# alexkroman/tiny-audio

Measured on AMD Instinct MI355X. Metric: training audio-sec/sec on 10s@16kHz clips, higher is better.
Workload: dtype bf16

## Files before the change

### include/ta355.h

```cpp
#ifndef TA355_H
#define TA355_H

#ifdef __cplusplus
extern "C" {
#endif

#ifndef __HIP_PLATFORM_AMD__
typedef struct ihipStream_t* hipStream_t;
#endif

#define TA_OK 0
#define TA_ERR_ARG 1
#define TA_ERR_LAUNCH 2

int ta_version(void);



long ta_logmel_scratch_floats(int B, int Ls, int n_mels);
int ta_logmel_mel_ranges(const float* melfb, int n_mels, int* mel_ranges, hipStream_t st);
int ta_logmel_f32(const float* wav, const long* lens, int B, int Ls, const float* dft, const float* window,
                  const float* melfb, int n_mels, float* feats, int* mask, float* scratch, const int* mel_ranges, hipStream_t st);

typedef struct {
// ... 199 lines not shown
int ta_lm_forward_loss_ex(const ta_lm_weights* w, const long* ids, const int* src_row, const float* audio,
                          const int* kmask, const int* pos, int B, int L, const int* label_rows,
                          const long* label_targets, int n_label_rows, float loss_scale, float* loss,
                          float* nll_rows, void* logits_out, void* tape, void* ws, long ws_bytes,
                          const ta_lora_dropout* drop, hipStream_t st);
int ta_lm_backward_ex(const ta_lm_weights* w, const int* src_row, const int* kmask, const int* pos, int B, int L,
                      const int* label_rows, int n_label_rows, float* d_audio, long n_audio_rows, float* d_embeds,
                      const ta_lm_lora_grads* lora_grads, const ta_lm_wgrads* wgrads, const long* ids, const void* tape, void* ws,
                      long ws_bytes, const ta_lora_dropout* drop, hipStream_t st);
int ta_lora_dropout_keep(const ta_lora_dropout* drop, int layer, int linear, int M, int in, unsigned char* out, hipStream_t st);


int ta_attention_enc_fwd(const void* qkv, void* out, int B, int heads, int S, hipStream_t st);

int ta_gemm_bf16_nt(const void* A, const void* W, void* C, int M, int N, int K, long lda, int a_rpb, long a_bs,
                    long ldc, int c_rpb, long c_bs, long c_off, const float* bias, const float* residual, int act,
                    int out_bf16, int splits, float* splitk_ws, hipStream_t st);
int ta_gemm_bf16_nt_ex(const void* A, const void* W, void* C, int M, int N, int K, long lda, int a_rpb, long a_bs,
                       long ldc, int c_rpb, long c_bs, long c_off, const float* bias, const float* residual, int act,
                       int out_bf16, int splits, float* splitk_ws, const int* a_idx, const int* seg,
                       const int* krange, hipStream_t st);
typedef struct {
  const void* a2; const void* w2; int k2; long lda2;
  const void* residual_bf16;
  const float* rope_tab; int rope_rows;
  int w_blocked;
  int rope_cols;
} ta_gemm_opts;
int ta_gemm_bf16_nt_opt(const void* A, const void* W, void* C, int M, int N, int K, long lda, int a_rpb, long a_bs,
                        long ldc, int c_rpb, long c_bs, long c_off, const float* bias, const float* residual, int act,
                        int out_bf16, int splits, float* splitk_ws, const int* a_idx, const int* seg,
                        const int* krange, const ta_gemm_opts* opts, hipStream_t st);
long ta_gemm_splitk_ws_bytes(int M, int N, int splits);
int ta_gemm_bf16_nt_grouped(const void* A, const void* W, void* C, int M, int N, int K, const float* bias, int act, int out_bf16,
                            const int* a_idx, const int* seg, const int* krange, int n_groups, long w_stride, long c_stride,
                            hipStream_t st);
long ta_gemm_bf16_tn_ws_bytes(int M, int Ny, int Nx);
int ta_gemm_bf16_tn(const void* Y, const void* X, float* out, int M, int Ny, int Nx, int accumulate, void* ws, long ws_bytes,
                    hipStream_t st);
int ta_profile_gemm(int enable);
int ta_profile_gemm_collect(double* total_ms, double* total_flops, long* launches);
long ta_profile_gemm_log(long* out, long max_rows);
int ta_gemm_reload_knobs(void);

int ta_layernorm_f32(const float* x, const float* w, const float* b, void* y_bf16, float* y_f32,
                     const float* rowscale, int M, int H, float eps, hipStream_t st);
int ta_layernorm_bf16(const void* x_bf16, const float* w, const float* b, void* y_bf16, float* y_f32, const float* rowscale,
                      int M, int H, float eps, hipStream_t st);
int ta_rmsnorm_fwd(const float* x, const float* w, void* y_bf16, float* y_f32, float* rstd, int M, int H,
                   float eps, int act_gelu, hipStream_t st);
int ta_rmsnorm_bwd(const float* dy, const float* x, const float* rstd, const float* w, const float* dres,
                   float* dx_f32, void* dx_bf16, float* dw_accum, int M, int H, int act_gelu, hipStream_t st);
int ta_rmsnorm_fwd_bf16(const void* x_bf16, const float* w, void* y_bf16, float* y_f32, float* rstd, int M, int H, float eps,
                        hipStream_t st);
int ta_rmsnorm_bwd_bf16(const void* dy, int dy_is_bf16, const void* x_bf16, const float* rstd, const float* w,
                        const float* dres, float* dx_f32, void* dx_bf16, int M, int H, hipStream_t st);
int ta_rmsnorm_bwd_bf16s(const void* dy, int dy_is_bf16, const void* x_bf16, const float* rstd, const float* w,
                         const void* dres_bf16, float* dx_f32, void* dx_bf16, int M, int H, hipStream_t st);
int ta_rmsnorm_bwd_dyb(const void* dy_bf16, const float* x, const float* rstd, const float* w, const float* dres, float* dx_f32,
                       void* dx_bf16, int M, int H, hipStream_t st);

int ta_rmsnorm_dw(const void* dy, int dy_is_bf16, const void* x, int x_is_bf16, const float* rstd, float* dw_accum, int M,
                  int H, hipStream_t st);

int ta_attention_fwd(const void* Q, const void* K, const void* VT, void* O, float* LSE, const int* kmask, int B,
                     int Hq, int Hkv, int L, int Lp, int head_dim, int causal, float scale, hipStream_t st);
// ... 66 lines not shown
```

### tiny_audio_amd/csrc/api.hip

```cpp
#include <cstdlib>
#include "common.h"
#include "internal.h"
#include "../../include/ta355.h"

extern "C" int ta_version(void) { return 4; }

#include <algorithm>
#include "host_util.h"


namespace {
struct EncDesc {
  int H, F, L, nh, NM, max_pos, k1;
  float eps;
  const void *conv1_w, *conv2_w;
  const float *conv1_b, *conv2_b, *norm_w, *norm_b;
  const float *rope_cos, *rope_sin, *rope_il, *pos_emb;
  const ta_enc_layer* layers;
  int res_f32;
  bool whisper;
};
EncDesc enc_desc(const ta_encoder_weights* w) {
  return EncDesc{w->hidden, w->ffn, w->n_layers, w->heads, w->n_mels, w->max_pos, 3 * w->n_mels, w->ln_eps, w->conv1_w, w->conv2_w,
                 w->conv1_b, w->conv2_b, w->norm_w, w->norm_b, w->rope_cos, w->rope_sin, w->rope_il, nullptr, w->layers, w->res_f32, false};
// ... 101 lines not shown
                                          void* out_bf16, float* out_f32, void* ws, long ws_bytes, hipStream_t st) {
  return enc_forward(enc_desc(w), feats, B, T, frame_keep, out_bf16, out_f32, ws, ws_bytes, st);
}

namespace {
struct MlpTape { float *h1, *r1, *h2, *r2; bf16_t* a1; size_t bytes; };
MlpTape mlp_tape(const ta_mlp_weights* w, int B, int S, void* base) {
  const int N = (S - w->k) / w->k + 1;
  const long Mp = (long)B * N;
  Carver c(base);
  MlpTape t;
  t.h1 = c.take<float>((size_t)Mp * w->hidden);
  t.r1 = c.take<float>((size_t)Mp);
  t.a1 = c.take<bf16_t>((size_t)Mp * w->hidden);
  t.h2 = c.take<float>((size_t)Mp * w->llm_dim);
  t.r2 = c.take<float>((size_t)Mp);
  t.bytes = c.total();
  return t;
}
struct MlpBwdWs { float *dh2, *da1, *skws, *dgws; bf16_t *dh2b, *dh2T, *a1T, *dh1b, *dh1T, *xsT; size_t bytes; };
MlpBwdWs mlp_bwd_ws(const ta_mlp_weights* w, int B, int S, void* base) {
  const int N = (S - w->k) / w->k + 1, Hd = w->hidden, D = w->llm_dim, In = w->k * w->enc_dim;
  const long Mp = (long)B * N; const int Kp = pad64((int)Mp);
  Carver c(base);
  MlpBwdWs s;
  s.dh2 = c.take<float>((size_t)Mp * D);
  s.dh2b = c.take<bf16_t>((size_t)Mp * D);
  s.dh2T = c.take<bf16_t>((size_t)D * Kp);
  s.a1T = c.take<bf16_t>((size_t)Hd * Kp);
  s.da1 = c.take<float>((size_t)Mp * Hd);
  s.dh1b = c.take<bf16_t>((size_t)Mp * Hd);
  s.dh1T = c.take<bf16_t>((size_t)Hd * Kp);
  s.xsT = c.take<bf16_t>((size_t)In * Kp);
  const int s1 = pick_splits(Hd, In, Kp), s2 = pick_splits(D, Hd, Kp);
  const size_t sk1 = (size_t)ta_gemm_splitk_ws_bytes(Hd, In, s1), sk2 = (size_t)ta_gemm_splitk_ws_bytes(D, Hd, s2);
  s.skws = c.take<float>((sk1 > sk2 ? sk1 : sk2) / 4 + 4);
  s.dgws = c.take<float>((size_t)ta_i_rmsnorm_bwd_ws_floats((int)Mp, Hd > D ? Hd : D));
  s.bytes = c.total();
  return s;
}
}

extern "C" long ta_mlp_tape_bytes(const ta_mlp_weights* w, int B, int S) { return (long)mlp_tape(w, B, S, nullptr).bytes; }
extern "C" long ta_mlp_bwd_workspace_bytes(const ta_mlp_weights* w, int B, int S) {
  return (long)mlp_bwd_ws(w, B, S, nullptr).bytes;
}

extern "C" int ta_mlp_projector_forward(const ta_mlp_weights* w, const void* x, int B, int S, float* y, void* tape,
                                        hipStream_t st) {
  const int k = w->k, E = w->enc_dim, Hd = w->hidden, D = w->llm_dim, In = k * E;
  const int N = (S - k) / k + 1;
  if (B <= 0 || N <= 0) return TA_OK;
  if (In % 64 || Hd % 64 || D % 4 || Hd % 4) return TA_ERR_ARG;
  const int Mp = B * N;
  MlpTape t = mlp_tape(w, B, S, tape);
  RC(ta_gemm_bf16_nt(x, w->w1, t.h1, Mp, Hd, In, In, N, (long)S * E, Hd, 0, 0, 0, nullptr, nullptr, 0, 0, 1, nullptr, st));
  RC(ta_rmsnorm_fwd(t.h1, w->g1, t.a1, nullptr, t.r1, Mp, Hd, w->eps, 1, st));
  RC(gemm(t.a1, w->w2, t.h2, Mp, D, Hd, nullptr, nullptr, 0, 0, st));
  RC(ta_rmsnorm_fwd(t.h2, w->g2, nullptr, y, t.r2, Mp, D, w->eps, 0, st));
  return TA_OK;
}

extern "C" int ta_mlp_projector_backward(const ta_mlp_weights* w, const void* x, int B, int S, const float* dy,
                                         const void* tape, float* dW1, float* dg1, float* dW2, float* dg2, void* ws,
                                         long ws_bytes, hipStream_t st) {
  const int k = w->k, E = w->enc_dim, Hd = w->hidden, D = w->llm_dim, In = k * E;
  const int N = (S - k) / k + 1;
// ... 65 lines not shown
    p.r_post = c.take<float>((size_t)d.M);
    p.gu = c.take<bf16_t>((size_t)d.M * 2 * d.F);
    if (w->lora_rank > 0 || w->train_base) {
      p.xn_s = c.take<bf16_t>((size_t)d.M * d.D); p.xn2_s = c.take<bf16_t>((size_t)d.M * d.D);
      p.act_s = c.take<bf16_t>((size_t)d.M * d.F);
    }
    if (w->lora_rank > 0) {
      p.xa_qkv = c.take<bf16_t>((size_t)d.M * 64); p.xa_o = c.take<bf16_t>((size_t)d.M * 64);
      p.xa_gu = c.take<bf16_t>((size_t)d.M * 64); p.xa_d = c.take<bf16_t>((size_t)d.M * 64);
      auto img = [&](LoraImg& g, int in, int N) {
        g.a = c.take<bf16_t>((size_t)64 * in); g.at = c.take<bf16_t>((size_t)64 * in);
        g.b = c.take<bf16_t>((size_t)64 * N); g.bt = c.take<bf16_t>((size_t)64 * N);
      };
      img(p.i_qkv, d.D, d.NQKV); img(p.i_o, d.nq * d.hd, d.D); img(p.i_gu, d.D, 2 * d.F); img(p.i_d, d.F, d.D);
    }
  }
  t.x_final = c.take<float>((size_t)d.M * d.D);
  t.r_f = c.take<float>((size_t)d.M);
  t.hn = c.take<bf16_t>((size_t)d.M * d.D);
  t.dlogits = c.take<bf16_t>((size_t)(n_lab > 0 ? n_lab : 1) * w->vocab_pad);
  t.bytes = c.total();
  return t;
}
struct LmWs {
  bf16_t *xn, *act, *hl, *dxb, *dact, *dgu, *dao, *dot, *dq, *dk, *dv, *dqkv, *dyB;
  float* lora_part;
  long lp_layer, lp_off[8], lp_size[8]; int lp_chunks[8];
  float *logits, *dhl, *dhn, *dxa, *dxb32, *dxn, *delta, *skws;
  bf16_t *tA, *tB;
  float* wsk;
  size_t bytes;
};
inline int wgrad_splits(int n_out, int k_in, int kp) { return pick_splits(n_out, k_in, kp); }
LmWs lm_ws(const ta_lm_weights* w, int B, int L, int n_lab, void* base) {
  const LmDims d = lm_dims(w, B, L);
  const int nl = n_lab > 0 ? n_lab : 1;
  Carver c(base);
  LmWs s;
  s.xn = c.take<bf16_t>((size_t)d.M * d.D);
  s.act = c.take<bf16_t>((size_t)d.M * d.F);
  s.hl = c.take<bf16_t>((size_t)nl * d.D);
  s.logits = c.take<float>((size_t)nl * w->vocab_pad);
  s.dhl = c.take<float>((size_t)nl * d.D);
  s.dhn = c.take<float>((size_t)d.M * d.D);
  s.dxa = c.take<float>((size_t)d.M * d.D);
  s.dxb32 = c.take<float>((size_t)d.M * d.D);
  s.dxn = c.take<float>((size_t)d.M * d.D);
  s.dxb = c.take<bf16_t>((size_t)d.M * d.D);
  s.dact = c.take<bf16_t>((size_t)d.M * d.F);
  s.dgu = c.take<bf16_t>((size_t)d.M * 2 * d.F);
  s.dao = c.take<bf16_t>((size_t)d.M * d.nq * d.hd);
  s.dot = nullptr;
  s.delta = c.take<float>((size_t)B * d.nq * L);
  s.dq = c.take<bf16_t>((size_t)d.M * d.nq * d.hd);
  s.dk = c.take<bf16_t>((size_t)d.M * d.nkv * d.hd);
  s.dv = c.take<bf16_t>((size_t)d.M * d.nkv * d.hd);
  s.dqkv = c.take<bf16_t>((size_t)d.M * d.NQKV);
  s.dyB = c.take<bf16_t>((size_t)d.M * 64);
  s.lora_part = nullptr; s.lp_layer = 0;
  if (w->lora_rank > 0) {
    const int r = w->lora_rank, bq = d.nq * d.hd;
    const int members[4] = {3, 1, 2, 1}, Ng[4] = {d.NQKV, d.D, 2 * d.F, d.D}, ing[4] = {d.D, bq, d.D, d.F};
    long off = 0;
    for (int g = 0; g < 4; ++g) {
      const int chunks = ta_cdiv((int)d.M, ta_i_lora_tn2_rows((int)d.M, Ng[g], ing[g]));
      s.lp_size[2 * g] = (long)members[g] * r * ing[g]; s.lp_size[2 * g + 1] = (long)Ng[g] * r;
      for (int h = 0; h < 2; ++h) { s.lp_chunks[2 * g + h] = chunks; s.lp_off[2 * g + h] = off; off += s.lp_size[2 * g + h] * chunks; }
    }
    s.lp_layer = off;
    s.lora_part = c.take<float>((size_t)off * w->n_layers);
  }
  const int sp = pick_splits(nl, d.D, w->vocab_pad);
  s.skws = c.take<float>((size_t)ta_gemm_splitk_ws_bytes(nl, d.D, sp) / 4 + 4);
  s.tA = s.tB = nullptr; s.wsk = nullptr;
  if (w->train_base) {
    const int Kp = pad64((int)d.M), Kl = pad64(nl), bq = d.nq * d.hd;
    const size_t a_rows = (size_t)std::max(std::max(2 * d.F, d.NQKV), d.D), b_rows = (size_t)std::max(std::max(d.F, bq), d.D);
    s.tA = c.take<bf16_t>(std::max(a_rows * Kp, (size_t)w->vocab_pad * Kl));
    s.tB = c.take<bf16_t>(std::max(b_rows * Kp, (size_t)d.D * Kl));
    const int shp[4][2] = {{d.NQKV, d.D}, {d.D, bq}, {2 * d.F, d.D}, {d.D, d.F}};
    size_t mx = 0;
    for (auto& q : shp) {
      mx = std::max(mx, (size_t)ta_gemm_splitk_ws_bytes(q[0], q[1], wgrad_splits(q[0], q[1], Kp)));
      mx = std::max(mx, (size_t)ta_gemm_bf16_tn_ws_bytes((int)d.M, q[0], q[1]));
    }
    s.wsk = c.take<float>(mx / 4 + 4);
  }
  s.bytes = c.total();
  return s;
}
}

extern "C" long ta_lm_tape_bytes(const ta_lm_weights* w, int B, int L, int n_label_rows) {
  LmLayerTape store[MAX_LM_LAYERS];
  if (w->n_layers > MAX_LM_LAYERS) return -1;
  return (long)lm_tape(w, B, L, n_label_rows, nullptr, store).bytes;
}
extern "C" long ta_lm_workspace_bytes(const ta_lm_weights* w, int B, int L, int n_label_rows) {
  return (long)lm_ws(w, B, L, n_label_rows, nullptr).bytes;
}

static int lm_layers_forward(const ta_lm_weights* w, const LmDims& d, int B, int L, const int* kmask, const int* pos,
                             LmLayerTape* store, bool alias, float* x_final, LmWs& s, const ta_i_lora_layer_imgs* ext,
                             bf16_t* kcache, bf16_t* vcache, int Lmax, hipStream_t st, const LoraDropDev* drop = nullptr) {
  const int M = (int)d.M;
  const float scale = 1.0f / sqrtf((float)d.hd);
  const bool lora = w->lora_rank > 0;
  const int r = w->lora_rank;
  if (lora && (r < 1 || 3 * r > 64)) return TA_ERR_ARG;
  const int lgm = lora ? (w->lora_groups ? w->lora_groups : 15) : 0;
  ta_gemm_opts kx = opts_none();
  auto lora_fwd = [&](const bf16_t* x, int in, const LoraImg& g, bf16_t* xa, int members, int lj0) -> int {
    if (drop) RC(ta_i_lora_skinny_nt_drop(x, in, g.a, xa, M, LoraDrop{*drop, (unsigned)lj0, r, members}, st));
    else RC(ta_i_lora_skinny_nt(x, in, g.a, xa, M, members * r, st));
    kx = opts_kext(xa, g.b);
    return TA_OK;
// ... 371 lines not shown
```

### tiny_audio_amd/csrc/gemm.hip

```cpp
#include "gemm_common.h"

template <int ACT, bool OUT_BF16, bool HAS_RES, int BMT = 128, bool KEXT = false>
__global__ __launch_bounds__(256, 2) void gemm_nt_kernel(GemmArgs p) {
  constexpr int MI = BMT / 32, WR = BMT / 2;
  __shared__ __attribute__((aligned(16))) char smem[4 * TILE_BYTES];
  const int tid = threadIdx.x, lane = tid & 63, wave = tid >> 6;
  const int wm = wave >> 1, wn = wave & 1;
  const int g = lane >> 4, l15 = lane & 15;

  const int nwg = gridDim.x;
  int bid = blockIdx.x;
  {
    const int q = nwg >> 3, r = nwg & 7, xcd = bid & 7, within = bid >> 3;
    bid = (xcd < r ? xcd * (q + 1) : r * (q + 1) + (xcd - r) * q) + within;
  }
  const int tiles = p.tiles_m * p.tiles_n;
  const int z = bid / tiles;
  int t = bid - z * tiles;
  const int GROUP_M = p.group_m > 0 ? p.group_m : 8;
  const int width = GROUP_M * p.tiles_n;
  const int group = t / width;
  const int first_m = group * GROUP_M;
  const int gsize = min(p.tiles_m - first_m, GROUP_M);
  int pm = first_m + (t % width) % gsize;
// ... 316 lines not shown
    for (int i = 0; i < NB; ++i) glds16_s(wb, w_off[i], base + A_BYTES + i * 8192);
    a_base += a_step; w_base += w_step;
  };
  auto first_dma = [&](const TileCtx& c, int st) {
    const int te = fresh_tid(), lr = te >> 3, clog = (te & 7) ^ ((lr >> 1) & 7);
    if (a_blk) {
#pragma unroll
      for (int i = 0; i < NA; ++i) a_off[i] = (unsigned)((((long)(i * nkt) << 12) + (lr << 6) + clog * 8) * 2);
      a_base = (const char*)(p.A + ((((long)((c.rbase + c.m0) >> 6)) * nkt + c.kb) << 12));
    } else if (p.a_plain) {
#pragma unroll
      for (int i = 0; i < NA; ++i)
        a_off[i] = (unsigned)(((long)(min(c.m0 + i * 64 + lr, c.Mact - 1) - c.m0) * p.lda + clog * 8) * 2);
      a_base = (const char*)(p.A + (long)(c.rbase + c.m0) * p.lda) + (long)c.kb * (BK * 2);
    } else {
#pragma unroll
      for (int i = 0; i < NA; ++i) {
        const int gm = c.rbase + min(c.m0 + i * 64 + lr, c.Mact - 1);
        a_off[i] = (unsigned)(((long)(gm / p.a_rpb) * p.a_bs + (long)(gm % p.a_rpb) * p.lda + clog * 8) * 2);
      }
      a_base = (const char*)p.A + (long)c.kb * (BK * 2);
    }
#pragma unroll
    for (int i = 0; i < NB; ++i) {
      const int gn = min(c.n0 + i * 64 + lr, p.N - 1);
      w_off[i] = p.w_blocked ? (unsigned)(((((long)((gn >> 6) - (c.n0 >> 6)) * nkt) << 12) + ((gn & 63) << 6) + clog * 8) * 2)
                             : (unsigned)(((long)(gn - c.n0) * p.K + clog * 8) * 2);
    }
    w_base = (const char*)c.Wp + (p.w_blocked ? (((long)(c.n0 >> 6) * nkt) << 13) + (long)c.kb * 8192 : ((long)c.n0 * p.K + (long)c.kb * BK) * 2);
    if (c.kb < c.ke) dma_tile(lds_w + st * STAGE);
  };
  constexpr bool GELU = ACT == 1;
  constexpr bool ROPE = ACT == 2;
  auto dma_epi = [&](const TileCtx& c, unsigned base) {
    const int te = fresh_tid();
    if (c.biasp && te < BN2 / 4) {
      const int n = c.n0 + te * 4;
      glds16_s(uniform_ptr((const char*)c.biasp), (unsigned)((n < p.N ? n : p.N - 4) * 4), base + EPI_LDS_BIAS);
    }
    if (GELU && !p.gelu_erf) {
      static_assert(GELU_LUT_N * 8 == 512 * 16, "one 16-B piece per thread");
      glds16_s(uniform_ptr((const char*)kGeluLut), (unsigned)(te * 16), base + EPI_LDS_TAB);
    }
    if (ROPE) {
      const char* rb = uniform_ptr((const char*)p.rope_tab);
#pragma unroll
      for (int i = 0; i < BM2 * 128 / 8192; ++i) {
        const int q = i * 512 + te, r = q >> 3, cch = q & 7;
        const int m = c.rbase + min(c.m0 + r, c.Mact - 1);
        glds16_s(rb, (unsigned)(((m % p.rope_rows) * 32 + ((cch ^ (r & 7)) << 2)) * 4), base + EPI_LDS_TAB + i * 8192);
      }
    }
  };

  const bool res_init = residual_is_start<ACT, OUT_BF16, HAS_RES>(p);
  int h = blockIdx.x;
  TileCtx cur = tile_ctx<BM2, BN2>(p, h, total);
  while (!cur.ok) {
    h += gridDim.x;
    if (h >= total) return;
    cur = tile_ctx<BM2, BN2>(p, h, total);
  }
  int ph = 0;
  first_dma(cur, ph);

  for (;;) {
    f32x4 acc[MI][NT];
    if (res_init) {
      const int te = fresh_tid();
      residual_start<MI, NT>(acc, p, cur.m0 + (te >> 8) * (BM2 / 2) + (te & 15), cur.Mact, cur.rbase, cur.n0 + ((te >> 6) & 3) * (BN2 / 4), (te >> 4) & 3);
    } else {
      zero_acc<MI, NT>(acc);
    }

    asm volatile("s_waitcnt vmcnt(0)" ::: "memory");
    __syncthreads();
    int hn = h + gridDim.x;
    TileCtx nx; nx.ok = 0;
    while (hn < total) {
      nx = tile_ctx<BM2, BN2>(p, hn, total);
      if (nx.ok) break;
      hn += gridDim.x;
    }
    if (lag) __builtin_amdgcn_s_barrier();
    for (int kt = cur.kb; kt < cur.ke; ++kt) {
      const int cs = ((kt - cur.kb) & 1) ^ ph;
      const bool more = kt + 1 < cur.ke;
      const char* S = smem + cs * STAGE;
      const unsigned nxt = lds_w + (cs ^ 1) * STAGE;
      bf16x8 af[MI], bfr[NT];
#pragma unroll
      for (int kk = 0; kk < 2; ++kk) {
        const int ko = kk ? koff1 : koff0;
#pragma unroll
        for (int j = 0; j < NT; ++j) bfr[j] = *(const bf16x8*)(S + b_rd + j * 2048 + ko);
#pragma unroll
        for (int i = 0; i < MI; ++i) af[i] = *(const bf16x8*)(S + a_rd + i * 2048 + ko);
        if (kk == 0) {
          if (more) {
            dma_tile(nxt);
          } else {
            dma_epi(cur, nxt);
          }
// ... 14 lines not shown
        __builtin_amdgcn_sched_barrier(0);
        __builtin_amdgcn_s_barrier();
        __builtin_amdgcn_sched_barrier(0);
      }
    }
    if (!lag) __builtin_amdgcn_s_barrier();

    const int nK = cur.ke - cur.kb;
    const int last = __builtin_amdgcn_readfirstlane(nK > 0 ? (((nK - 1) & 1) ^ ph) : ph);
    const char* els = smem + (last ^ 1) * STAGE;
    if (nK <= 0) {
      dma_epi(cur, lds_w + (last ^ 1) * STAGE);
      asm volatile("s_waitcnt vmcnt(0)" ::: "memory");
      __syncthreads();
    }
    if (nx.ok) first_dma(nx, last);
    const float2* lut = (GELU && !p.gelu_erf) ? (const float2*)(els + EPI_LDS_TAB) : nullptr;

    const int te = fresh_tid();
    const int e_l15 = te & 15, e_g = (te >> 4) & 3, e_wn = (te >> 6) & 3, e_wm = te >> 8;
    char* Cb = (char*)p.C;
    if (p.splits > 1) Cb += (long)cur.z * p.slab_stride * 4;
    const bool wide = epilogue_wide_ok(p);
    const int erow0 = e_wm * (BM2 / 2) + e_l15;
    const bool full = OUT_BF16 && wide && p.c_plain && (!HAS_RES || res_init) && cur.m0 + BM2 <= cur.Mact && cur.n0 + BN2 <= p.N;
    if constexpr (OUT_BF16) {
      if (full) epilogue_tile_full<MI, NT, ACT, true>(acc, p, Cb, cur.m0 + erow0, cur.rbase, cur.n0 + e_wn * (BN2 / 4), e_g, cur.biasp, lut, els, cur.n0, erow0);
    }
    if (full) { }
    else if (res_init)
      epilogue_tile<MI, NT, ACT, OUT_BF16, false, 0, true>(acc, p, Cb, cur.m0 + erow0, cur.Mact, cur.rbase, cur.n0 + e_wn * (BN2 / 4), e_g,
                                                           wide, cur.biasp, lut, els, cur.n0, erow0);
    else
      epilogue_tile<MI, NT, ACT, OUT_BF16, HAS_RES, ((BM2 == 192 || (HAS_RES && !OUT_BF16 && ACT == 0)) ? 1 : 0), true>(acc, p, Cb, cur.m0 + erow0, cur.Mact, cur.rbase,
                                                                                cur.n0 + e_wn * (BN2 / 4), e_g, wide, cur.biasp, lut, els, cur.n0, erow0);
    if (!nx.ok) return;
    cur = nx; h = hn; ph = last;
  }
}



__global__ void splitk_reduce_kernel(const float* __restrict__ slabs, int splits, long slab_stride, const float* add,
                                     float* out, bf16_t* __restrict__ out_bf, long n4) {
  for (long i = (long)blockIdx.x * blockDim.x + threadIdx.x; i < n4; i += (long)gridDim.x * blockDim.x) {
    float4 s = add ? ((const float4*)add)[i] : make_float4(0.f, 0.f, 0.f, 0.f);
    for (int z = 0; z < splits; ++z) {
      const float4 v = ((const float4*)(slabs + (long)z * slab_stride))[i];
      s.x += v.x; s.y += v.y; s.z += v.z; s.w += v.w;
    }
    if (out) ((float4*)out)[i] = s;
    if (out_bf) {
      uint2 o; o.x = pack2bf(s.x, s.y); o.y = pack2bf(s.z, s.w);
      ((uint2*)out_bf)[i] = o;
    }
  }
}

template <int N> __device__ __forceinline__ void wait_vm_lgkm0_n() { asm volatile("s_waitcnt vmcnt(%0) lgkmcnt(0)" ::"n"(N) : "memory"); }
template <int ACT, bool OUT_BF16, bool HAS_RES, bool KEXT = false>
__global__ __launch_bounds__(256) void gemm_nt_kernel_v5(GemmArgs p) {
  constexpr int BM5 = 192, BN5 = 128, NS = 3;
  constexpr int A_BYTES = BM5 * 128, SLOT = (BM5 + BN5) * 128;
  __shared__ __attribute__((aligned(16))) char smem[NS * SLOT];
  const int tid = threadIdx.x, lane = tid & 63, wave = tid >> 6;
  const int wm = wave >> 1, wn = wave & 1;
  const int g = lane >> 4, l15 = lane & 15;
// ... 129 lines not shown
      }
      __builtin_amdgcn_s_setprio(0);
      if (FIRST) advance(); else rslot = nslot;
    };
    for (int kt = 0; kt < nt; ++kt) {
      step(std::true_type{}, af0, bf0, af1, bf1);
      step(std::false_type{}, af1, bf1, af0, bf0);
    }
    asm volatile("s_waitcnt vmcnt(0)" ::: "memory");
  }

  char* Cb = (char*)p.C;
  if (p.splits > 1) Cb += (long)z * p.slab_stride * 4;
  const bool wide = epilogue_wide_ok(p);
  const float2* lut = stage_gelu_lut<ACT, 256>(smem, p, tid, true);
  if (res_init) epilogue_tile<6, 4, ACT, OUT_BF16, false>(acc, p, Cb, m0 + wm * 96 + l15, Mact, rbase, n0 + wn * 64, g, wide, biasp, lut);
  else epilogue_tile<6, 4, ACT, OUT_BF16, HAS_RES, ((HAS_RES && !OUT_BF16) ? 3 : 2)>(acc, p, Cb, m0 + wm * 96 + l15, Mact, rbase, n0 + wn * 64, g, wide, biasp, lut);
}

#include <vector>
namespace {
struct ProfRec { hipEvent_t a, b; double flops; };
bool g_prof_on = false;
std::vector<ProfRec> g_prof;
#define TA_GEMM_LOG_FIELDS 24
bool g_log_on = false;
std::vector<long> g_log;
}

#include <cstdlib>
struct GemmKnobs {
  int variant;
  int gelu_erf;
  void load() {
    auto i = [](const char* n, int d) { const char* v = getenv(n); return (v && *v) ? atoi(v) : d; };
    variant = i("TA355_GEMM_VARIANT", -1);
    gelu_erf = i("TA355_GELU_LUT", 1) == 0;
  }
};
static GemmKnobs& knobs() {
  static GemmKnobs k = [] { GemmKnobs x; x.load(); return x; }();
  return k;
}
void ta_i_reload_decode_knobs();
extern "C" int ta_gemm_reload_knobs(void) { knobs().load(); ta_i_reload_decode_knobs(); return TA_OK; }

static int pick_variant(int M, int N, int K, int splits) {
  const int forced = knobs().variant;
  if (forced >= 0 && forced <= 12 && !(forced >= 6 && forced <= 9) && forced != 11) return forced;
  const double rate[6] = {1.0, TA355_RATE_256x256, TA355_RATE_256x128, TA355_RATE_256x256_PP, TA355_RATE_256x320_PP, TA355_RATE_96x128};
  const int bm[6] = {128, 256, 256, 256, 256, 96}, bn[6] = {128, 256, 128, 256, 320, 128}, slots[6] = {512, 256, 256, 256, 256, 512};
  int best = 0; double best_t = 1e300;
  for (int v = 0; v < 6; ++v) {
    const long tiles = (long)ta_cdiv(M, bm[v]) * ta_cdiv(N, bn[v]) * splits;
    const double rounds = (double)((tiles + slots[v] - 1) / slots[v]);
    const double t = rounds * (double)bm[v] * bn[v] / rate[v] * ((v == 0 || v == 5) ? 2.0 : 1.0);
    if (t < best_t) { best_t = t; best = v; }
  }
  {
    const long tiles = (long)ta_cdiv(M, 192) * ta_cdiv(N, 128) * splits;
    const double t = (double)((tiles + 255) / 256) * 192.0 * 128.0 / TA355_RATE_192x128;
    if (TA355_RATE_192x128 > 0.0 && K / splits >= 2048 && t < best_t) { best_t = t; best = 10; }
  }
  {
    const long tiles = (long)ta_cdiv(M, 192) * ta_cdiv(N, 256) * splits;
    const double t = (double)((tiles + 255) / 256) * 192.0 * 256.0 / TA355_RATE_192x256_PP;
    if (TA355_RATE_192x256_PP > 0.0 && K / splits >= 128 && t < best_t) { best_t = t; best = 12; }
  }
  return best;
}

template <int ACT, bool OUT_BF16, bool HAS_RES, bool KEXT>
static void launch_variant(int variant, bool persist, int grid, int pgrid, const GemmArgs& a, hipStream_t st) {
  if (variant == 0) TA_LAUNCH((gemm_nt_kernel<ACT, OUT_BF16, HAS_RES, 128, KEXT>), dim3(grid), dim3(256), 0, st, a);
  else if (variant == 5) TA_LAUNCH((gemm_nt_kernel<ACT, OUT_BF16, HAS_RES, 96, KEXT>), dim3(grid), dim3(256), 0, st, a);
  else if (variant == 1) TA_LAUNCH((gemm_nt_kernel_v2<256, ACT, OUT_BF16, HAS_RES, false, KEXT>), dim3(grid), dim3(512), 0, st, a);
  else if (variant == 12) TA_LAUNCH((gemm_nt_kernel_v4<256, ACT, OUT_BF16, HAS_RES, 192>), dim3(pgrid), dim3(512), 0, st, a);
  else if (variant == 3 && persist) TA_LAUNCH((gemm_nt_kernel_v4<256, ACT, OUT_BF16, HAS_RES>), dim3(pgrid), dim3(512), 0, st, a);
  else if (variant == 4 && persist) TA_LAUNCH((gemm_nt_kernel_v4<320, ACT, OUT_BF16, HAS_RES>), dim3(pgrid), dim3(512), 0, st, a);
  else if (variant == 3) TA_LAUNCH((gemm_nt_kernel_v2<256, ACT, OUT_BF16, HAS_RES, true, KEXT>), dim3(grid), dim3(512), 0, st, a);
  else if (variant == 4) TA_LAUNCH((gemm_nt_kernel_v2<320, ACT, OUT_BF16, HAS_RES, true, KEXT>), dim3(grid), dim3(512), 0, st, a);
  else if (variant == 10) TA_LAUNCH((gemm_nt_kernel_v5<ACT, OUT_BF16, HAS_RES, KEXT>), dim3(grid), dim3(256), 0, st, a);
  else TA_LAUNCH((gemm_nt_kernel_v2<128, ACT, OUT_BF16, HAS_RES, false, KEXT>), dim3(grid), dim3(512), 0, st, a);
}

template <int ACT, bool OUT_BF16, bool HAS_RES>
static int launch_gemm(GemmArgs a, hipStream_t st) {
  if (a.A2 && ACT != 0) return TA_ERR_ARG;
  int variant = pick_variant(a.M, a.N, a.K, a.splits);
  const bool a_far = !a.a_plain && ((long)(a.M / a.a_rpb + 1) * a.a_bs + a.lda * a.a_rpb) * 2 >= (1L << 32);
  if (variant == 10 && (a.w_blocked || a.a_idx || a_far)) variant = 5;
  if (variant == 12 && (a.a_idx || a_far || a.A2)) variant = 3;
  const int bm = variant == 0 ? 128 : (variant == 5 ? 96 : ((variant == 10 || variant == 12) ? 192 : 256));
  const int bn = variant == 4 ? 320 : ((variant == 1 || variant == 3 || variant == 12) ? 256 : 128);
  a.tiles_m = ta_cdiv(a.M, bm) + ((a.grp_n > 0 && a.seg) ? a.grp_n : 0); a.tiles_n = ta_cdiv(a.N, bn);
  const int grid = a.tiles_m * a.tiles_n * a.splits;
  a.group_m = (variant != 0 && a.tiles_m <= 8) ? a.tiles_m : 0;
  a.wide = (((long)a.N | a.ldc | a.c_off | a.c_bs) & 7) == 0;
  a.gelu_erf = knobs().gelu_erf;
  const bool persist = (variant == 3 || variant == 4) && !a.a_idx && !a.A2 && !a_far;
  static const int ncu = [] { int dev = 0, n = 0; (void)hipGetDevice(&dev); (void)hipDeviceGetAttribute(&n, hipDeviceAttributeMultiprocessorCount, dev); return n > 0 ? n : 256; }();
  const int pgrid = grid < ncu ? grid : ncu;
  ProfRec r;
  if (g_prof_on) {
    if (hipEventCreate(&r.a) != hipSuccess || hipEventCreate(&r.b) != hipSuccess) return TA_ERR_LAUNCH;
    r.flops = 2.0 * (double)a.M * (double)a.N * (double)a.K;
    (void)hipEventRecord(r.a, st);
  }
  if constexpr (ACT == 0) {
    if (a.A2) launch_variant<ACT, OUT_BF16, HAS_RES, true>(variant, persist, grid, pgrid, a, st);
  }
  if (!a.A2) launch_variant<ACT, OUT_BF16, HAS_RES, false>(variant, persist, grid, pgrid, a, st);
  if (g_prof_on) { (void)hipEventRecord(r.b, st); g_prof.push_back(r); }
  if (g_log_on) {
    const long flags = (a.a_idx ? 1 : 0) | (a.seg ? 2 : 0) | (a.krange ? 4 : 0) | (a.A2 ? 8 : 0) | (a.w_blocked ? 16 : 0) | (a.grp_n > 0 ? 32 : 0) |
                       (a.a_plain ? 256 : 0) | (a.c_plain ? 512 : 0);
    const long rec[TA_GEMM_LOG_FIELDS] = {a.M, a.N, a.K, a.lda, a.a_rpb, a.a_bs, a.ldc, a.c_rpb, a.c_bs, a.c_off, ACT, OUT_BF16 ? 1 : 0,
                                          HAS_RES ? 1 : 0, a.res_bf16, a.bias ? 1 : 0, a.splits, a.rope_cols, a.rope_rows, flags, a.K2, variant,
                                          a.grp_n, 0, persist ? 1 : 0};
    g_log.insert(g_log.end(), rec, rec + TA_GEMM_LOG_FIELDS);
  }
  TA_CHECK_LAUNCH();
  return TA_OK;
}

extern "C" int ta_profile_gemm(int enable) {
  g_prof_on = enable == 1;
// ... 143 lines not shown
```

### tiny_audio_amd/csrc/gemm_common.h

```cpp
#pragma once
#include "common.h"
#include "../../include/ta355.h"
#include <type_traits>

struct GemmArgs {
  const bf16_t* A;
  const bf16_t* W;
  void* C;
  const float* bias;
  const float* res;
  int M, N, K;
  long lda; int a_rpb; long a_bs;
  long ldc; int c_rpb; long c_bs; long c_off;
  int tiles_m, tiles_n, splits;
  long slab_stride;
  const int* a_idx;
  const int* seg;
  const int* krange;
  const bf16_t* A2; const bf16_t* W2; int K2; long lda2;
  int res_bf16;
  const float* rope_tab; int rope_rows; int rope_cols;
  int group_m;
  int wide;
  int w_blocked;
  int a_plain, c_plain;
  int gelu_erf;
  int a_blocked;
  int grp_n; long grp_w_stride;
};

#define BM 128
#define BN 128
#define BK 64
#ifndef TA355_RATE_256x256
#define TA355_RATE_256x256 0.9
#define TA355_RATE_256x128 0.5
#define TA355_RATE_256x256_PP 1.40
#define TA355_RATE_96x128 0.93
#define TA355_RATE_192x128 1.1
#define TA355_RATE_192x256_PP 1.15
#define TA355_RATE_256x320_PP 1.42
#endif
#define TILE_BYTES (BM * BK * 2)
#include "gelu_lut.h"

__device__ __forceinline__ void glds16_s(const char* base, unsigned off, unsigned lds) {
  asm volatile("s_mov_b32 m0, %0\n\ts_nop 0\n\tglobal_load_lds_dwordx4 %1, %2" ::"s"(lds), "v"(off), "s"(base) : "memory");
}
__device__ __forceinline__ const char* uniform_ptr(const char* q) {
  const unsigned long v = (unsigned long)q;
  const unsigned lo = __builtin_amdgcn_readfirstlane((unsigned)v), hi = __builtin_amdgcn_readfirstlane((unsigned)(v >> 32));
  return (const char*)(((unsigned long)hi << 32) | lo);
}
__device__ __forceinline__ void glds16(const void* g, void* l) {
  __builtin_amdgcn_global_load_lds((const __attribute__((address_space(1))) void*)g,
                                   (__attribute__((address_space(3))) void*)l, 16, 0, 0);
}

__device__ __forceinline__ float gelu_lut(float x, const float2* lut) {
  float t = fmaf(x, GELU_LUT_SCALE, GELU_LUT_BIAS);
  t = __builtin_amdgcn_fmed3f(t, 0.f, (float)(GELU_LUT_N - 1));
  const float2 e = lut[(int)t];
  return fmaf(e.x, x, e.y);
}
#define EPI_LDS_BIAS 0
#define EPI_LDS_TAB 2048
__device__ __forceinline__ int opaque_sgpr(int v) { asm volatile("" : "+s"(v)); return v; }
template <int NT> struct EpiPre { uint2 r[NT]; };
template <int NT, int ACT, bool OUT_BF16, bool HAS_RES, bool ELS = false>
__device__ __forceinline__ void epilogue_strip(const f32x4* acc, const GemmArgs& p, char* Cb, long roff, int nb, int g, bool wide,
                                               int m, const float* bias, const float2* lut = nullptr, const EpiPre<NT>* pre = nullptr,
                                               bool pre_r = false, const char* els = nullptr, int ecol0 = 0, int erow = 0,
                                               uint2* oret = nullptr, const float4* pref = nullptr) {
  static_assert(ACT >= 0 && ACT <= 2, "epilogue form");
  constexpr int BASE = ACT;
// ... 65 lines not shown
  }
}
template <int MI, int NT, int ACT, bool ELS>
__device__ __forceinline__ void epilogue_tile_full(const f32x4 (*acc)[NT], const GemmArgs& p, char* Cb, int ml0, int rbase, int nb, int g,
                                                   const float* bias, const float2* lut, const char* els, int ecol0, int erow0) {
  static_assert(NT >= 4, "two column pairs per strip");
  const int l15 = ml0 & 15;
  const long own0 = p.c_off + (long)(rbase + ml0) * p.ldc;
  const long step = 16L * p.ldc;
  const int colx = nb + (l15 >> 3) * 32 + 16 * (g & 1) + 8 * (g >> 1);
  char* px = Cb + (p.c_off + (long)(rbase + ml0 - (l15 & 8)) * p.ldc + colx) * 2;
  char* py = px + 16L * p.ldc;
#pragma unroll
  for (int i = 0; i < MI; ++i) {
    uint2 o[NT];
    epilogue_strip<NT, ACT, true, false, ELS>(acc[i], p, Cb, own0 + i * step, nb, g, true, rbase + ml0 + i * 16, bias, lut, nullptr, false, els,
                                              ecol0, erow0 + i * 16, o);
    uint32_t q[2][4];
#pragma unroll
    for (int pp = 0; pp < 2; ++pp) {
      const auto a = __builtin_amdgcn_permlane16_swap(o[2 * pp].x, o[2 * pp + 1].x, false, false);
      const auto b = __builtin_amdgcn_permlane16_swap(o[2 * pp].y, o[2 * pp + 1].y, false, false);
      q[pp][0] = a[0]; q[pp][1] = b[0]; q[pp][2] = a[1]; q[pp][3] = b[1];
    }
    uint32_t x[4], y[4];
#pragma unroll
    for (int d = 0; d < 4; ++d) {
      x[d] = __builtin_amdgcn_update_dpp(q[0][d], q[1][d], 0x128, 0xf, 0xc, false);
      y[d] = __builtin_amdgcn_update_dpp(q[1][d], q[0][d], 0x128, 0xf, 0x3, false);
    }
    *(uint4*)(px + i * step * 2) = make_uint4(x[0], x[1], x[2], x[3]);
    *(uint4*)(py + i * step * 2) = make_uint4(y[0], y[1], y[2], y[3]);
#pragma unroll
    for (int j = 4; j < NT; ++j) *(uint2*)(Cb + (own0 + i * step + nb + j * 16 + g * 4) * 2) = o[j];
  }
}
template <int MI, int NT, int ACT, bool OUT_BF16, bool HAS_RES, int AHEAD = 0, bool ELS = false, int PIN = 0>
__device__ __forceinline__ void epilogue_tile(const f32x4 (*acc)[NT], const GemmArgs& p, char* Cb, int ml0, int Mact, int rbase, int nb,
                                              int g, bool wide, const float* bias, const float2* lut, const char* els = nullptr,
                                              int ecol0 = 0, int erow0 = 0) {
  const int c_rpb_o = opaque_sgpr(p.c_rpb);
  auto row_off = [&](int m) -> long {
    return p.c_off + (p.c_plain ? (long)m * p.ldc : (long)(m / c_rpb_o) * p.c_bs + (long)(m % c_rpb_o) * p.ldc);
  };
  int ncl[NT];
#pragma unroll
  for (int j = 0; j < NT; ++j) {
    const int n = nb + j * 16 + g * 4;
    ncl[j] = n < p.N ? n : p.N - 4;
  }
  const bool pre_r = AHEAD > 0 && HAS_RES && p.res_bf16;
  auto fetch = [&](int i, uint2* dst) {
    int ml = ml0 + i * 16; if (ml >= Mact) ml = Mact - 1;
    const long ro = row_off(rbase + ml);
#pragma unroll
    for (int j = 0; j < NT; ++j) dst[j] = *(const uint2*)((const bf16_t*)p.res + ro + ncl[j]);
  };
  auto strip = [&](int i, const EpiPre<NT>* pre) {
    const int ml = ml0 + i * 16;
    if constexpr (PIN > 0) {
#pragma unroll
      for (int j = 0; j < NT; ++j)
        if (j < PIN) asm volatile("" : "+a"(const_cast<f32x4&>(acc[i][j])));
    }
    if (ml < Mact) {
      const int m = rbase + ml;
      epilogue_strip<NT, ACT, OUT_BF16, HAS_RES, ELS>(acc[i], p, Cb, row_off(m), nb, g, wide, m, bias, lut, pre, pre_r, els, ecol0, erow0 + i * 16);
// ... 187 lines not shown
```

### tiny_audio_amd/csrc/host_util.h

```cpp
#pragma once
#include "common.h"
#include "internal.h"
#include "../../include/ta355.h"

namespace {
struct Carver {
  char* base; size_t off;
  explicit Carver(void* b) : base((char*)b), off(0) {}
  template <typename T> T* take(size_t n) {
    off = (off + 255) & ~(size_t)255;
    T* p = base ? (T*)(base + off) : nullptr;
    off += n * sizeof(T);
    return p;
  }
  size_t total() const { return (off + 255) & ~(size_t)255; }
};
inline int pad64(int x) { return (x + 63) / 64 * 64; }
inline int gemm(const void* A, const void* W, void* C, int M, int N, int K, const float* bias, const float* res, int act,
                int out_bf16, hipStream_t st) {
  return ta_gemm_bf16_nt(A, W, C, M, N, K, K, 0, 0, N, 0, 0, 0, bias, res, act, out_bf16, 1, nullptr, st);
}
inline int gemm_opt(const void* A, const void* W, void* C, int M, int N, int K, const float* bias, const float* res, int act,
                    int out_bf16, const ta_gemm_opts& o, hipStream_t st) {
  return ta_gemm_bf16_nt_opt(A, W, C, M, N, K, K, 0, 0, N, 0, 0, 0, bias, res, act, out_bf16, 1, nullptr, nullptr, nullptr, nullptr,
                             &o, st);
}
inline ta_gemm_opts opts_none() { return ta_gemm_opts{nullptr, nullptr, 0, 0, nullptr, nullptr, 0, 0, 0}; }
inline ta_gemm_opts opts_kext(const void* a2, const void* w2) { ta_gemm_opts o = opts_none(); o.a2 = a2; o.w2 = w2; o.k2 = 64; o.lda2 = 64; return o; }
inline int pick_splits(int M, int N, int K) {
  const long tiles = (long)ta_cdiv(M, 128) * ta_cdiv(N, 128);
  int s = 1;
  while (tiles * s < 512 && K / 64 / (s * 2) >= 8 && s < 64) s *= 2;
  return s;
}
#define RC(x) do { int rc__ = (x); if (rc__) return rc__; } while (0)
inline size_t lora_imgs_carve(const ta_lm_weights* w, void* base, ta_i_lora_layer_imgs* out) {
  Carver c(base);
  const int D = w->hidden, F = w->ffn, bq = w->heads * w->head_dim, NQKV = (w->heads + 2 * w->kv_heads) * w->head_dim;
  const int in[4] = {D, bq, D, F}, N[4] = {NQKV, D, 2 * F, D};
  for (int l = 0; l < w->n_layers; ++l)
    for (int g = 0; g < 4; ++g) {
      LoraImg im;
      im.a = c.take<bf16_t>((size_t)64 * in[g]); im.at = c.take<bf16_t>((size_t)64 * in[g]);
      im.b = c.take<bf16_t>((size_t)64 * N[g]); im.bt = c.take<bf16_t>((size_t)64 * N[g]);
      if (out) out[l].g[g] = im;
    }
  return c.total();
}
}
```

### tiny_audio_amd/ops.py

```python
from __future__ import annotations

import ctypes as C

import torch

from . import _lib
from ._lib import check, lib

BF16 = torch.bfloat16
F32 = torch.float32


def ptr(t):
    return None if t is None else C.c_void_p(t.data_ptr())


def stream():
    if _lib.DRY_RUN:
        return None
    return C.c_void_p(torch.cuda.current_stream().cuda_stream)


def _req(t, dtype=None):
    assert (t.is_cuda or _lib.DRY_RUN) and t.is_contiguous(), "ta355 ops need contiguous CUDA(HIP) tensors"
    if dtype is not None:
        assert t.dtype == dtype, (t.dtype, dtype)
    return t


_KNOB_KEYS = ("TA355_GEMM_VARIANT", "TA355_GELU_LUT", "TA355_DECODE_FUSED")
_knob_state = None


def sync_gemm_knobs():
    global _knob_state
    import os
    cur = tuple(os.environ.get(k) for k in _KNOB_KEYS)
    if cur != _knob_state:
        if _knob_state is not None or any(v is not None for v in cur):
            lib().ta_gemm_reload_knobs()
        _knob_state = cur


def gemm_nt(A, W, M=None, N=None, K=None, *, out=None, out_dtype=BF16, bias=None, residual=None, act=0,
            a_map=None, c_map=None, splits=1, k_ext=None, residual_bf16=None, rope=None, w_blocked=False):
    _req(A, BF16); _req(W, BF16)
    sync_gemm_knobs()
    opts = None
    if residual_bf16 is not None or k_ext is not None or rope is not None or w_blocked:
        from ._lib import GemmOpts
        opts = GemmOpts()
        opts.w_blocked = int(bool(w_blocked))
        if rope is not None:
            _req(rope[0], F32)
            opts.rope_tab, opts.rope_rows = ptr(rope[0]), int(rope[1])
            opts.rope_cols = int(rope[2]) if len(rope) > 2 else 0
        if residual_bf16 is not None:
            _req(residual_bf16, BF16)
            opts.residual_bf16 = ptr(residual_bf16)
        if k_ext is not None:
            A2, W2 = k_ext
            _req(A2, BF16); _req(W2, BF16)
            opts.a2, opts.w2, opts.k2, opts.lda2 = ptr(A2), ptr(W2), W2.shape[1], A2.shape[1]
# ... 378 lines not shown
```

Before: 7660.

## Jointly plan split-K and tile variant with cost model; add 192x384 tile

Replaces the fixed split-K heuristic with a planner that searches split count and tile variant together, using a cost model that includes per-tile K overhead and split-K reduction cost. Adds a new 192x384 persistent tile variant, plus a wider residual load path and paired permlane16 swaps so the epilogue writes 16-byte bf16 stores. Workspace sizing now uses the maximum split any variant could pick. This trades more tuning complexity and extra template instantiations for better occupancy and less reduction overhead on the GEMMs; the old rule stays available behind an environment knob.

```diff
diff --git a/include/ta355.h b/include/ta355.h
--- a/include/ta355.h
+++ b/include/ta355.h
@@ -255,6 +255,7 @@
                         int out_bf16, int splits, float* splitk_ws, const int* a_idx, const int* seg,
                         const int* krange, const ta_gemm_opts* opts, hipStream_t st);
 long ta_gemm_splitk_ws_bytes(int M, int N, int splits);
+int ta_gemm_plan_splits(int M, int N, int K, int* variant_out, int* max_splits);
 int ta_gemm_bf16_nt_grouped(const void* A, const void* W, void* C, int M, int N, int K, const float* bias, int act, int out_bf16,
                             const int* a_idx, const int* seg, const int* krange, int n_groups, long w_stride, long c_stride,
                             hipStream_t st);
diff --git a/tiny_audio_amd/csrc/api.hip b/tiny_audio_amd/csrc/api.hip
--- a/tiny_audio_amd/csrc/api.hip
+++ b/tiny_audio_amd/csrc/api.hip
@@ -157,7 +157,7 @@
   s.dh1b = c.take<bf16_t>((size_t)Mp * Hd);
   s.dh1T = c.take<bf16_t>((size_t)Hd * Kp);
   s.xsT = c.take<bf16_t>((size_t)In * Kp);
-  const int s1 = pick_splits(Hd, In, Kp), s2 = pick_splits(D, Hd, Kp);
+  const int s1 = pick_splits_ws(Hd, In, Kp), s2 = pick_splits_ws(D, Hd, Kp);
   const size_t sk1 = (size_t)ta_gemm_splitk_ws_bytes(Hd, In, s1), sk2 = (size_t)ta_gemm_splitk_ws_bytes(D, Hd, s2);
   s.skws = c.take<float>((sk1 > sk2 ? sk1 : sk2) / 4 + 4);
   s.dgws = c.take<float>((size_t)ta_i_rmsnorm_bwd_ws_floats((int)Mp, Hd > D ? Hd : D));
@@ -289,6 +289,7 @@
   size_t bytes;
 };
 inline int wgrad_splits(int n_out, int k_in, int kp) { return pick_splits(n_out, k_in, kp); }
+inline int wgrad_splits_ws(int n_out, int k_in, int kp) { return pick_splits_ws(n_out, k_in, kp); }
 LmWs lm_ws(const ta_lm_weights* w, int B, int L, int n_lab, void* base) {
   const LmDims d = lm_dims(w, B, L);
   const int nl = n_lab > 0 ? n_lab : 1;
@@ -327,7 +328,7 @@
     s.lp_layer = off;
     s.lora_part = c.take<float>((size_t)off * w->n_layers);
   }
-  const int sp = pick_splits(nl, d.D, w->vocab_pad);
+  const int sp = pick_splits_ws(nl, d.D, w->vocab_pad);
   s.skws = c.take<float>((size_t)ta_gemm_splitk_ws_bytes(nl, d.D, sp) / 4 + 4);
   s.tA = s.tB = nullptr; s.wsk = nullptr;
   if (w->train_base) {
@@ -338,7 +339,7 @@
     const int shp[4][2] = {{d.NQKV, d.D}, {d.D, bq}, {2 * d.F, d.D}, {d.D, d.F}};
     size_t mx = 0;
     for (auto& q : shp) {
-      mx = std::max(mx, (size_t)ta_gemm_splitk_ws_bytes(q[0], q[1], wgrad_splits(q[0], q[1], Kp)));
+      mx = std::max(mx, (size_t)ta_gemm_splitk_ws_bytes(q[0], q[1], wgrad_splits_ws(q[0], q[1], Kp)));
       mx = std::max(mx, (size_t)ta_gemm_bf16_tn_ws_bytes((int)d.M, q[0], q[1]));
     }
     s.wsk = c.take<float>(mx / 4 + 4);
diff --git a/tiny_audio_amd/csrc/gemm.hip b/tiny_audio_amd/csrc/gemm.hip
--- a/tiny_audio_amd/csrc/gemm.hip
+++ b/tiny_audio_amd/csrc/gemm.hip
@@ -372,6 +372,7 @@
   };
   constexpr bool GELU = ACT == 1;
   constexpr bool ROPE = ACT == 2;
+  constexpr bool WIDE_RES = HAS_RES && NT > 5;
   auto dma_epi = [&](const TileCtx& c, unsigned base) {
     const int te = fresh_tid();
     if (c.biasp && te < BN2 / 4) {
@@ -408,7 +409,7 @@
     f32x4 acc[MI][NT];
     if (res_init) {
       const int te = fresh_tid();
-      residual_start<MI, NT>(acc, p, cur.m0 + (te >> 8) * (BM2 / 2) + (te & 15), cur.Mact, cur.rbase, cur.n0 + ((te >> 6) & 3) * (BN2 / 4), (te >> 4) & 3);
+      residual_start<MI, NT, WIDE_RES ? 2 : 0>(acc, p, cur.m0 + (te >> 8) * (BM2 / 2) + (te & 15), cur.Mact, cur.rbase, cur.n0 + ((te >> 6) & 3) * (BN2 / 4), (te >> 4) & 3);
     } else {
       zero_acc<MI, NT>(acc);
     }
@@ -489,7 +490,7 @@
       epilogue_tile<MI, NT, ACT, OUT_BF16, false, 0, true>(acc, p, Cb, cur.m0 + erow0, cur.Mact, cur.rbase, cur.n0 + e_wn * (BN2 / 4), e_g,
                                                            wide, cur.biasp, lut, els, cur.n0, erow0);
     else
-      epilogue_tile<MI, NT, ACT, OUT_BF16, HAS_RES, ((BM2 == 192 || (HAS_RES && !OUT_BF16 && ACT == 0)) ? 1 : 0), true>(acc, p, Cb, cur.m0 + erow0, cur.Mact, cur.rbase,
+      epilogue_tile<MI, NT, ACT, OUT_BF16, HAS_RES, (((BM2 == 192 && !WIDE_RES) || (HAS_RES && !OUT_BF16 && ACT == 0)) ? 1 : 0), true>(acc, p, Cb, cur.m0 + erow0, cur.Mact, cur.rbase,
                                                                                 cur.n0 + e_wn * (BN2 / 4), e_g, wide, cur.biasp, lut, els, cur.n0, erow0);
     if (!nx.ok) return;
     cur = nx; h = hn; ph = last;
@@ -685,10 +686,12 @@
 struct GemmKnobs {
   int variant;
   int gelu_erf;
+  int old_splits;
   void load() {
     auto i = [](const char* n, int d) { const char* v = getenv(n); return (v && *v) ? atoi(v) : d; };
     variant = i("TA355_GEMM_VARIANT", -1);
     gelu_erf = i("TA355_GELU_LUT", 1) == 0;
+    old_splits = i("TA355_SPLITK_RULE", 1) == 0;
   }
 };
 static GemmKnobs& knobs() {
@@ -698,37 +701,81 @@
 void ta_i_reload_decode_knobs();
 extern "C" int ta_gemm_reload_knobs(void) { knobs().load(); ta_i_reload_decode_knobs(); return TA_OK; }
 
+namespace {
+struct TileVariant { int id, bm, bn, slots; double rate; int min_k; };
+const TileVariant kTileVariants[] = {
+    {0, 128, 128, 512, 1.0, 0},
+    {1, 256, 256, 256, TA355_RATE_256x256, 0},
+    {2, 256, 128, 256, TA355_RATE_256x128, 0},
+    {3, 256, 256, 256, TA355_RATE_256x256_PP, 0},
+    {4, 256, 320, 256, TA355_RATE_256x320_PP, 0},
+    {5, 96, 128, 512, TA355_RATE_96x128, 0},
+    {10, 192, 128, 256, TA355_RATE_192x128, 2048},
+    {12, 192, 256, 256, TA355_RATE_192x256_PP, 128},
+    {13, 192, 384, 256, TA355_RATE_192x384_PP, 128},
+};
+bool variant_in_library(int v) { return v >= 0 && v <= 13 && !(v >= 6 && v <= 9) && v != 11; }
+double variant_cost(const TileVariant& v, int M, int N, int K, int splits) {
+  const long tiles = (long)ta_cdiv(M, v.bm) * ta_cdiv(N, v.bn) * splits;
+  const double rounds = (double)((tiles + v.slots - 1) / v.slots);
+  const int nkt = K / BK;
+  double t = rounds * (double)v.bm * v.bn / v.rate * (v.slots == 512 ? 2.0 : 1.0) * (double)(ta_cdiv(nkt, splits) + TA355_TILE_OVERHEAD_KT);
+  if (splits > 1) t += TA355_SPLITK_REDUCE_COST * (double)(splits + 1) * (double)M * (double)N;
+  return t;
+}
+bool variant_offered(const TileVariant& v, int K, int splits) { return v.rate > 0.0 && (v.min_k == 0 || K / splits >= v.min_k); }
+}
+
 static int pick_variant(int M, int N, int K, int splits) {
   const int forced = knobs().variant;
-  if (forced >= 0 && forced <= 12 && !(forced >= 6 && forced <= 9) && forced != 11) return forced;
-  const double rate[6] = {1.0, TA355_RATE_256x256, TA355_RATE_256x128, TA355_RATE_256x256_PP, TA355_RATE_256x320_PP, TA355_RATE_96x128};
-  const int bm[6] = {128, 256, 256, 256, 256, 96}, bn[6] = {128, 256, 128, 256, 320, 128}, slots[6] = {512, 256, 256, 256, 256, 512};
+  if (variant_in_library(forced)) return forced;
   int best = 0; double best_t = 1e300;
-  for (int v = 0; v < 6; ++v) {
-    const long tiles = (long)ta_cdiv(M, bm[v]) * ta_cdiv(N, bn[v]) * splits;
-    const double rounds = (double)((tiles + slots[v] - 1) / slots[v]);
-    const double t = rounds * (double)bm[v] * bn[v] / rate[v] * ((v == 0 || v == 5) ? 2.0 : 1.0);
-    if (t < best_t) { best_t = t; best = v; }
-  }
-  {
-    const long tiles = (long)ta_cdiv(M, 192) * ta_cdiv(N, 128) * splits;
-    const double t = (double)((tiles + 255) / 256) * 192.0 * 128.0 / TA355_RATE_192x128;
-    if (TA355_RATE_192x128 > 0.0 && K / splits >= 2048 && t < best_t) { best_t = t; best = 10; }
-  }
-  {
-    const long tiles = (long)ta_cdiv(M, 192) * ta_cdiv(N, 256) * splits;
-    const double t = (double)((tiles + 255) / 256) * 192.0 * 256.0 / TA355_RATE_192x256_PP;
-    if (TA355_RATE_192x256_PP > 0.0 && K / splits >= 128 && t < best_t) { best_t = t; best = 12; }
+  for (const TileVariant& v : kTileVariants) {
+    if (!variant_offered(v, K, splits)) continue;
+    const double t = variant_cost(v, M, N, K, splits);
+    if (t < best_t) { best_t = t; best = v.id; }
   }
   return best;
 }
 
+extern "C" int ta_gemm_plan_splits(int M, int N, int K, int* variant_out, int* max_splits) {
+  int best_v = 0, best_s = 1, mx = 1;
+  double best_t = 1e300;
+  if (knobs().old_splits) {
+    const long tiles = (long)ta_cdiv(M, 128) * ta_cdiv(N, 128);
+    while (tiles * best_s < 512 && K / 64 / (best_s * 2) >= 8 && best_s < 64) best_s *= 2;
+    best_v = pick_variant(M, N, K, best_s);
+    mx = best_s;
+  } else if (M > 0 && N > 0 && K >= BK) {
+    const int forced = knobs().variant;
+    const int nkt = K / BK;
+    int s_hi = nkt / 8; if (s_hi > 64) s_hi = 64; if (s_hi < 1) s_hi = 1;
+    for (const TileVariant& v : kTileVariants) {
+      int vs = 1; double vt = 1e300;
+      for (int s = 1; s <= s_hi; ++s) {
+        if (!variant_offered(v, K, s)) continue;
+        const double t = variant_cost(v, M, N, K, s);
+        if (t < vt) { vt = t; vs = s; }
+      }
+      if (vs > mx) mx = vs;
+      if (variant_in_library(forced) ? v.id == forced : vt < best_t) { best_t = vt; best_v = v.id; best_s = vs; }
+    }
+  }
+  if (variant_out) *variant_out = best_v;
+  if (max_splits) *max_splits = mx;
+  return best_s;
+}
+
+template <int ACT, bool OUT_BF16, bool HAS_RES> constexpr bool kNo192x384 = ACT == 1 && OUT_BF16 && HAS_RES;
 template <int ACT, bool OUT_BF16, bool HAS_RES, bool KEXT>
 static void launch_variant(int variant, bool persist, int grid, int pgrid, const GemmArgs& a, hipStream_t st) {
   if (variant == 0) TA_LAUNCH((gemm_nt_kernel<ACT, OUT_BF16, HAS_RES, 128, KEXT>), dim3(grid), dim3(256), 0, st, a);
   else if (variant == 5) TA_LAUNCH((gemm_nt_kernel<ACT, OUT_BF16, HAS_RES, 96, KEXT>), dim3(grid), dim3(256), 0, st, a);
   else if (variant == 1) TA_LAUNCH((gemm_nt_kernel_v2<256, ACT, OUT_BF16, HAS_RES, false, KEXT>), dim3(grid), dim3(512), 0, st, a);
   else if (variant == 12) TA_LAUNCH((gemm_nt_kernel_v4<256, ACT, OUT_BF16, HAS_RES, 192>), dim3(pgrid), dim3(512), 0, st, a);
+  else if (variant == 13) {
+    if constexpr (!kNo192x384<ACT, OUT_BF16, HAS_RES>) TA_LAUNCH((gemm_nt_kernel_v4<384, ACT, OUT_BF16, HAS_RES, 192>), dim3(pgrid), dim3(512), 0, st, a);
+  }
   else if (variant == 3 && persist) TA_LAUNCH((gemm_nt_kernel_v4<256, ACT, OUT_BF16, HAS_RES>), dim3(pgrid), dim3(512), 0, st, a);
   else if (variant == 4 && persist) TA_LAUNCH((gemm_nt_kernel_v4<320, ACT, OUT_BF16, HAS_RES>), dim3(pgrid), dim3(512), 0, st, a);
   else if (variant == 3) TA_LAUNCH((gemm_nt_kernel_v2<256, ACT, OUT_BF16, HAS_RES, true, KEXT>), dim3(grid), dim3(512), 0, st, a);
@@ -744,8 +791,9 @@
   const bool a_far = !a.a_plain && ((long)(a.M / a.a_rpb + 1) * a.a_bs + a.lda * a.a_rpb) * 2 >= (1L << 32);
   if (variant == 10 && (a.w_blocked || a.a_idx || a_far)) variant = 5;
   if (variant == 12 && (a.a_idx || a_far || a.A2)) variant = 3;
-  const int bm = variant == 0 ? 128 : (variant == 5 ? 96 : ((variant == 10 || variant == 12) ? 192 : 256));
-  const int bn = variant == 4 ? 320 : ((variant == 1 || variant == 3 || variant == 12) ? 256 : 128);
+  if (variant == 13 && (a.a_idx || a_far || a.A2 || kNo192x384<ACT, OUT_BF16, HAS_RES>)) variant = 4;
+  const int bm = variant == 0 ? 128 : (variant == 5 ? 96 : ((variant == 10 || variant == 12 || variant == 13) ? 192 : 256));
+  const int bn = variant == 13 ? 384 : (variant == 4 ? 320 : ((variant == 1 || variant == 3 || variant == 12) ? 256 : 128));
   a.tiles_m = ta_cdiv(a.M, bm) + ((a.grp_n > 0 && a.seg) ? a.grp_n : 0); a.tiles_n = ta_cdiv(a.N, bn);
   const int grid = a.tiles_m * a.tiles_n * a.splits;
   a.group_m = (variant != 0 && a.tiles_m <= 8) ? a.tiles_m : 0;
diff --git a/tiny_audio_amd/csrc/gemm_common.h b/tiny_audio_amd/csrc/gemm_common.h
--- a/tiny_audio_amd/csrc/gemm_common.h
+++ b/tiny_audio_amd/csrc/gemm_common.h
@@ -41,6 +41,13 @@
 #define TA355_RATE_192x256_PP 1.15
 #define TA355_RATE_256x320_PP 1.42
 #endif
+#ifndef TA355_RATE_192x384_PP
+#define TA355_RATE_192x384_PP 1.38
+#endif
+#ifndef TA355_TILE_OVERHEAD_KT
+#define TA355_TILE_OVERHEAD_KT 4
+#define TA355_SPLITK_REDUCE_COST 0.03
+#endif
 #define TILE_BYTES (BM * BK * 2)
 #include "gelu_lut.h"
 
@@ -172,7 +179,12 @@
     *(uint4*)(px + i * step * 2) = make_uint4(x[0], x[1], x[2], x[3]);
     *(uint4*)(py + i * step * 2) = make_uint4(y[0], y[1], y[2], y[3]);
 #pragma unroll
-    for (int j = 4; j < NT; ++j) *(uint2*)(Cb + (own0 + i * step + nb + j * 16 + g * 4) * 2) = o[j];
+    for (int j = 4; j + 1 < NT; j += 2) {
+      const auto a = __builtin_amdgcn_permlane16_swap(o[j].x, o[j + 1].x, false, false);
+      const auto b = __builtin_amdgcn_permlane16_swap(o[j].y, o[j + 1].y, false, false);
+      *(uint4*)(Cb + (own0 + i * step + nb + 16 * (j + (g & 1)) + 8 * (g >> 1)) * 2) = make_uint4(a[0], b[0], a[1], b[1]);
+    }
+    if (NT > 4 && (NT & 1)) *(uint2*)(Cb + (own0 + i * step + nb + (NT - 1) * 16 + g * 4) * 2) = o[NT - 1];
   }
 }
 template <int MI, int NT, int ACT, bool OUT_BF16, bool HAS_RES, int AHEAD = 0, bool ELS = false, int PIN = 0>
diff --git a/tiny_audio_amd/csrc/host_util.h b/tiny_audio_amd/csrc/host_util.h
--- a/tiny_audio_amd/csrc/host_util.h
+++ b/tiny_audio_amd/csrc/host_util.h
@@ -27,12 +27,8 @@
 }
 inline ta_gemm_opts opts_none() { return ta_gemm_opts{nullptr, nullptr, 0, 0, nullptr, nullptr, 0, 0, 0}; }
 inline ta_gemm_opts opts_kext(const void* a2, const void* w2) { ta_gemm_opts o = opts_none(); o.a2 = a2; o.w2 = w2; o.k2 = 64; o.lda2 = 64; return o; }
-inline int pick_splits(int M, int N, int K) {
-  const long tiles = (long)ta_cdiv(M, 128) * ta_cdiv(N, 128);
-  int s = 1;
-  while (tiles * s < 512 && K / 64 / (s * 2) >= 8 && s < 64) s *= 2;
-  return s;
-}
+inline int pick_splits(int M, int N, int K) { return ta_gemm_plan_splits(M, N, K, nullptr, nullptr); }
+inline int pick_splits_ws(int M, int N, int K) { int mx = 1; (void)ta_gemm_plan_splits(M, N, K, nullptr, &mx); return mx; }
 #define RC(x) do { int rc__ = (x); if (rc__) return rc__; } while (0)
 inline size_t lora_imgs_carve(const ta_lm_weights* w, void* base, ta_i_lora_layer_imgs* out) {
   Carver c(base);
diff --git a/tiny_audio_amd/ops.py b/tiny_audio_amd/ops.py
--- a/tiny_audio_amd/ops.py
+++ b/tiny_audio_amd/ops.py
@@ -28,7 +28,7 @@
     return t
 
 
-_KNOB_KEYS = ("TA355_GEMM_VARIANT", "TA355_GELU_LUT", "TA355_DECODE_FUSED")
+_KNOB_KEYS = ("TA355_GEMM_VARIANT", "TA355_GELU_LUT", "TA355_DECODE_FUSED", "TA355_SPLITK_RULE")
 _knob_state = None
 
 
```

Measured after the change: 7698 (median of 6 runs). No clear change (+0.5%).
